# ruc98/Distributed-Data-Parallel-ML-Training

Measured on AMD Instinct MI355X. Metric: images/sec (whole node) VGG-11 CIFAR-10, higher is better.
Workload: dtype bf16; 1 GPU; model=vgg11, global_batch=256, per_gpu_batch=256, parallelism=dp1, hipgraph=True, buckets=1, grad_comm=fp32, comm=inline, optimizer=SGD(lr=0.1, momentum=0.9, wd=1e-4) fused

## Files before the change

distributed-data-parallel-ml-training_amd/csrc/bind.cpp:

```cpp
#include <hip/hip_runtime.h>
#include <pybind11/pybind11.h>
#include <pybind11/stl.h>

#include <stdexcept>
#include <string>
#include <tuple>
#include <vector>

#include "runtime/comm.h"

namespace py = pybind11;
using ddp_amd::BucketSpec;
using ddp_amd::RcclComm;
using ddp_amd::Reducer;

#include "kernels/api.h"

template <typename T>
static T* P(uintptr_t v) { return reinterpret_cast<T*>(v); }
static hipStream_t S(uintptr_t v) { return reinterpret_cast<hipStream_t>(v); }
static void check(int rc, const char* what) {
  if (rc != 0) {
    std::string msg = std::string(what) + " failed: ";
    msg += (rc > 0) ? hipGetErrorString((hipError_t)rc) : "invalid arguments";
// ... 90 lines not shown
      py::tuple b = bn.cast<py::tuple>();
      f.gamma = P<float>(b[0].cast<uintptr_t>());
      f.beta = P<float>(b[1].cast<uintptr_t>());
      f.eps = b[2].cast<float>();
      f.relu = b[3].cast<int>();
      f.pool = b[4].cast<int>();
      f.coef = P<float>(b[5].cast<uintptr_t>());
      f.y = P<unsigned short>(b[6].cast<uintptr_t>());
      f.P = b[7].cast<int>();
      f.Q = b[8].cast<int>();
      fp = &f;
    }
    ddp_amd::TrFwdIn ti{};
    const ddp_amd::TrFwdIn* tp = nullptr;
    if (!fin.is_none()) {
      py::tuple b = fin.cast<py::tuple>();
      ti.z = P<unsigned short>(b[0].cast<uintptr_t>());
      ti.stats = P<float>(b[1].cast<uintptr_t>());
      ti.gamma = P<float>(b[2].cast<uintptr_t>());
      ti.beta = P<float>(b[3].cast<uintptr_t>());
      ti.eps = b[4].cast<float>();
      ti.relu = b[5].cast<int>();
      ti.pool = b[6].cast<int>();
      ti.coef = P<float>(b[7].cast<uintptr_t>());
      ti.y = P<unsigned short>(b[8].cast<uintptr_t>());
      tp = &ti;
    }
    int done = 0;
    const int rc = ddp_conv_fwd_tr(&c, P<void>(x), P<void>(wc), P<float>(bias), P<void>(z),
                                   P<float>(stats), P<float>(ws), ws_elems, fp, &done, tp, S(st));
    if (rc < 0) check(rc, "conv_fwd_tr");
    if (rc >= 2) check(rc - 2, "conv_fwd_tr");
    return rc == 1 ? 1 + done : 0;
  }, py::arg("g"), py::arg("x"), py::arg("wc"), py::arg("bias"), py::arg("z"), py::arg("stats"),
     py::arg("ws"), py::arg("ws_elems"), py::arg("st"), py::arg("bn") = py::none(),
     py::arg("fin") = py::none());
  m.def("l0_ok", [](py::tuple g) {
    auto c = geom(g);
    return ddp_l0_ok(&c) == 1;
  });
  m.def("l0_fwd", [](py::tuple g, uintptr_t x, uintptr_t wc, uintptr_t bias, float eps, int relu,
                     uintptr_t stats, uintptr_t gamma, uintptr_t beta, uintptr_t coef, uintptr_t y,
                     uintptr_t code, uintptr_t zw, uintptr_t st) {
    auto c = geom(g);
    ddp_amd::L0Io io{};
    io.zw = P<void>(zw);
    io.x = P<void>(x); io.wc = P<void>(wc); io.bias = P<float>(bias); io.eps = eps; io.relu = relu;
    io.stats = P<float>(stats); io.gamma = P<float>(gamma); io.beta = P<float>(beta);
    io.coef = P<float>(coef); io.y = P<void>(y); io.code = P<void>(code);
    check(ddp_l0_fwd(&c, &io, S(st)), "l0_fwd");
  });
  m.def("l0_bwd", [](py::tuple g, uintptr_t x, uintptr_t wc, uintptr_t bias, float eps, int relu,
                     uintptr_t coef, uintptr_t dy, uintptr_t sums, uintptr_t dz, uintptr_t dgamma,
                     uintptr_t dbeta, uintptr_t code, uintptr_t zw, uintptr_t st, int sums_ready) {
    auto c = geom(g);
    ddp_amd::L0Io io{};
    io.x = P<void>(x); io.wc = P<void>(wc); io.bias = P<float>(bias); io.eps = eps; io.relu = relu;
    io.coef = P<float>(coef); io.dy = P<void>(dy); io.sums = P<float>(sums); io.dz = P<void>(dz);
    io.dgamma = P<float>(dgamma); io.dbeta = P<float>(dbeta); io.code = P<void>(code);
    io.zw = P<void>(zw);
    io.sums_ready = sums_ready;
    check(ddp_l0_bwd(&c, &io, S(st)), "l0_bwd");
  }, py::arg("g"), py::arg("x"), py::arg("wc"), py::arg("bias"), py::arg("eps"), py::arg("relu"),
     py::arg("coef"), py::arg("dy"), py::arg("sums"), py::arg("dz"), py::arg("dgamma"),
     py::arg("dbeta"), py::arg("code"), py::arg("zw"), py::arg("stream"),
     py::arg("sums_ready") = 0);
  m.def("conv_tr_would_serve", [](py::tuple g, size_t ws_elems, int in_mode) {
    auto c = geom(g);
    return ddp_conv_tr_would_serve(&c, ws_elems, in_mode) == 1;
  });
  m.def("conv_tr_set", [](int mode, int M, int K, int C, int H, int bm, int bn, int splits,
                          int stages) { ddp_conv_tr_set(mode, M, K, C, H, bm, bn, splits, stages); },
        py::arg("mode"), py::arg("M"), py::arg("K"), py::arg("C"), py::arg("H"), py::arg("bm"),
        py::arg("bn"), py::arg("splits"), py::arg("stages") = 0);
  m.def("conv_tr_geometry", [](int BM, int N, int H, int W) {
    int o[7];
    ddp_conv_tr_geometry(BM, N, H, W, o);
    return std::vector<int>(o, o + 7);
  });
  m.def("linear_head_bwd_bn", [](uintptr_t dl, uintptr_t W, uintptr_t x, int B, int F, int J,
                                 uintptr_t g, py::tuple bn, py::tuple bna, uintptr_t dW,
                                 uintptr_t db, uintptr_t st) {
    ddp_amd::BnBwdFuse f{};
    f.z = P<unsigned short>(bn[0].cast<uintptr_t>());
    f.coef = P<float>(bn[1].cast<uintptr_t>());
    f.sums = P<float>(bn[2].cast<uintptr_t>());
    f.pool = bn[3].cast<int>();
    f.relu = bn[4].cast<int>();
    f.Hz = bn[5].cast<int>();
    f.Wz = bn[6].cast<int>();
    ddp_amd::BnBwdApply ap{};
    bn_apply(bna, &ap);
    const int rc = ddp_linear_head_bwd_bn(P<float>(dl), P<float>(W), P<void>(x), B, F, J,
                                          P<float>(g), &f, &ap, P<float>(dW), P<float>(db), S(st));
    if (rc < 0) check(rc, "linear_head_bwd_bn");
    if (rc >= 2) check(rc - 2, "linear_head_bwd_bn");
    return rc == 1;
  });
  m.def("conv_fwd_smallk", [](py::tuple g, uintptr_t x, uintptr_t wc, uintptr_t bias, uintptr_t y,
                              uintptr_t stats, uintptr_t st) {
    auto c = geom(g);
    const int rc = ddp_conv_fwd_smallk(&c, P<void>(x), P<void>(wc), P<float>(bias), P<void>(y),
                                       P<float>(stats), S(st));
    if (rc > 0) check(rc, "conv_fwd_smallk");
    return rc == 0;
  });
  m.def("conv_dgrad", [](py::tuple g, uintptr_t dy, uintptr_t wt, uintptr_t dx, uintptr_t ws,
                         size_t ws_elems, int splits, uintptr_t st, int accumulate, py::object bn,
                         py::object bna, uintptr_t acc_dy, uintptr_t acc_mask) {
    auto c = geom(g);
    if (acc_mask) {
      check(ddp_conv_dgrad_acc(&c, P<void>(dy), P<void>(wt), P<void>(dx), P<float>(ws), ws_elems,
                               splits, P<void>(acc_dy), P<unsigned char>(acc_mask), S(st)),
            "conv_dgrad_acc");
      return false;
    }
    if (bn.is_none()) {
      check(ddp_conv_dgrad(&c, P<void>(dy), P<void>(wt), P<void>(dx), P<float>(ws), ws_elems,
                           splits, accumulate, S(st)), "conv_dgrad");
// ... 490 lines not shown
```

distributed-data-parallel-ml-training_amd/csrc/kernels/api.h:

```cpp
#pragma once
#include <hip/hip_runtime.h>
#include <stddef.h>
#include <stdint.h>

namespace ddp_amd {

#ifdef DDP_AMD_DETERMINISTIC
constexpr int kStatRep = 4096;
constexpr bool kDeterministic = true;
#else
constexpr int kStatRep = 16;
constexpr bool kDeterministic = false;
#endif

struct ConvGeom {
  int N, H, W, C;
  int K;
  int R, S, stride, pad;
  int P, Q;
  int Creal;
  int wkrsc;
};

struct BnArgs {
// ... 61 lines not shown
  const float* beta;
  float eps;
  int relu, pool;
  float* coef;
  unsigned short* y;
};

struct HeadBnIn {
  const unsigned short* z;
  const float* stats;
  const float* gamma;
  const float* beta;
  float eps;
  int relu;
  float* coef;
  unsigned short* y;
};

struct LrSched {
  unsigned step;
  unsigned n;
  unsigned next;
  unsigned pad;
};

struct SgdFuse {
  float* p;
  float* buf;
  unsigned short* wc;
  float lr, momentum, wd, grad_scale;
  int nesterov;
  const LrSched* sched;
};

struct L0Io {
  const void* x;
  const void* wc;
  const float* bias;
  float eps;
  int relu;
  float* stats;
  const float* gamma;
  const float* beta;
  float* coef;
  void* y;
  const void* dy;
  float* sums;
  void* dz;
  void* code;
  void* zw;
  float* dgamma;
  float* dbeta;
  int sums_ready;
};

struct PackDesc {
  const float* p;
  unsigned short* wc;
  unsigned short* wt;
  int K, Cr, C, R, S;
  int krsc;
};

struct AugArgs {
  const unsigned char* images;
  const int* labels;
  const int* indices;
  const int* cursor;
  int L, B, H, W, Cp, pad, flip;
  uint32_t seed, epoch;
  float mean[3], inv_std[3];
  unsigned short* x;
  long long* y;
  float* zero;
  size_t zero_n;
  LrSched* sched;
};

}

extern "C" {
int ddp_conv_fwd(const ddp_amd::ConvGeom* g, const void* x, const void* wc, const float* bias,
                 void* y, float* stats, float* ws, size_t ws_elems, int splits, hipStream_t st);
int ddp_conv_fwd_bn(const ddp_amd::ConvGeom* g, const void* x, const void* wc, const float* bias,
                    void* z, float* stats, float* ws, size_t ws_elems, const ddp_amd::BnFwdFuse* bn,
                    hipStream_t st);
int ddp_conv_fwd_finish(const ddp_amd::ConvGeom* g, float* ws, int splits, const float* bias,
                        void* z, float* stats, const ddp_amd::BnFwdFuse* bn, int* bn_done,
                        hipStream_t st);
int ddp_conv_fwd_tr(const ddp_amd::ConvGeom* g, const void* x, const void* wc, const float* bias,
                    void* z, float* stats, float* ws, size_t ws_elems,
                    const ddp_amd::BnFwdFuse* bn, int* bn_done, const ddp_amd::TrFwdIn* in,
                    hipStream_t st);
int ddp_conv_tr_would_serve(const ddp_amd::ConvGeom* g, size_t ws_elems, int in_mode);
void ddp_conv_tr_set(int mode, int M, int K, int C, int H, int bm, int bn, int splits, int stages);
int ddp_conv_tr_geometry(int BM, int N, int H, int W, int* out7);
int ddp_linear_head_bwd_bn(const float* dl, const float* W, const void* x, int B, int F, int J,
                           const float* gscale, const ddp_amd::BnBwdFuse* bn,
                           const ddp_amd::BnBwdApply* ba, float* dW, float* db, hipStream_t st);
void ddp_conv_bn_fuse_rows(int rows);
int ddp_conv_dgrad(const ddp_amd::ConvGeom* g, const void* dy, const void* wt, void* dx,
                   float* ws, size_t ws_elems, int splits, int accumulate, hipStream_t st);
int ddp_conv_dgrad_acc(const ddp_amd::ConvGeom* g, const void* dy, const void* wt, void* dx,
                       float* ws, size_t ws_elems, int splits, const void* acc_dy,
                       const unsigned char* acc_mask, hipStream_t st);
int ddp_conv_dgrad_bn(const ddp_amd::ConvGeom* g, const void* dy, const void* wt, void* dx,
                      float* ws, size_t ws_elems, int splits, const ddp_amd::BnBwdFuse* bn,
                      const ddp_amd::BnBwdApply* ba, int* bn_done, hipStream_t st);
int ddp_conv_wgrad(const ddp_amd::ConvGeom* g, const void* dy, const void* x, float* dw,
                   float* ws, size_t ws_elems, int splits, hipStream_t st);
int ddp_bn_act_fwd(const ddp_amd::BnArgs* a, hipStream_t st);
int ddp_bn_act_bwd(const ddp_amd::BnArgs* a, hipStream_t st);
int ddp_bn_act_fwd_res(const ddp_amd::BnArgs* a, const ddp_amd::BnArgs* r, hipStream_t st);
int ddp_bn_act_bwd_res(const ddp_amd::BnArgs* a, hipStream_t st);
int ddp_bn_bwd_local_ok(int N, int H, int W, int C, int pool);
void ddp_bn_bwd_local_set(long long max_loads);
int ddp_bn_pool_linear_ce_fwd(const ddp_amd::HeadBnIn* bn, const float* W, const float* b,
                              const long long* labels, int B, int F, int J, float* dlogits,
                              float* loss_sum, int* correct, float* loss_acc, hipStream_t st);
int ddp_linear_ce_fwd(const void* x, const float* W, const float* b, const long long* labels,
                      int B, int F, int J, float* logits, float* dlogits, float* loss_sum,
                      int* correct, float* loss_acc, hipStream_t st);
int ddp_linear_bwd(const float* dlogits, const void* x, const float* W, int B, int F, int J,
                   const float* gscale, void* dx, float* dW, float* db, hipStream_t st);
int ddp_softmax_ce(const void* logits, int logits_bf16, const long long* labels, int B, int J,
                   float* loss_sum, int* correct, void* dlogits, int dlogits_bf16,
                   hipStream_t st);
int ddp_sgd(float* p, const float* g, float* buf, size_t n, float lr, float momentum, float wd,
            float grad_scale, int nesterov, const ddp_amd::LrSched* sched, hipStream_t st);
int ddp_conv_fwd_smallk(const ddp_amd::ConvGeom* g, const void* x, const void* wc,
                        const float* bias, void* y, float* stats, hipStream_t st);
void ddp_conv_options(int stages);
void ddp_conv_epi_stage_set(int on);
int ddp_bn_pool3_fwd(const ddp_amd::BnArgs* a, unsigned char* idx, hipStream_t st);
int ddp_bn_pool3_bwd(const ddp_amd::BnArgs* a, const unsigned char* idx, hipStream_t st);
void ddp_conv_pair_mode(int mode, int items);
void ddp_sgd_fuse_register(float* dw, const ddp_amd::SgdFuse* f, int clear);
void ddp_sgd_fuse_begin();
int ddp_l0_ok(const ddp_amd::ConvGeom* g);
int ddp_l0_fwd(const ddp_amd::ConvGeom* g, const ddp_amd::L0Io* io, hipStream_t st);
int ddp_l0_bwd(const ddp_amd::ConvGeom* g, const ddp_amd::L0Io* io, hipStream_t st);
int ddp_conv_wgrad_final(const ddp_amd::ConvGeom* g, const void* dy, const void* x, float* dw,
                         float* ws, size_t ws_elems, int splits, hipStream_t st);
int ddp_sgd_fuse_taken(uintptr_t* out, int cap);
int ddp_sgd_fuse_taken_master(uintptr_t* out, int cap);
void ddp_conv_pair_force(int splits_dg, int splits_wg, int tile);
int ddp_conv_bwd_pair(const ddp_amd::ConvGeom* g, const void* dy, const void* wc, void* dx,
                      const void* x, float* dw, float* ws, size_t ws_elems,
                      const ddp_amd::BnBwdFuse* bn, const ddp_amd::BnBwdApply* ba, int* bn_done,
                      hipStream_t st);
void ddp_conv_tune_set(int mode, int M, int N, int K, int tile, int splits, int stages);
void ddp_conv_pair_tune_set(int M, int N, int K, int hw, int tile, int sd, int sw);
void ddp_conv_wgrad_pm_set(int on);
void ddp_conv_rows_pm_set(int on);
void ddp_bn_fold_bwd_mb(int mb);
void ddp_bn_fold_grid(int blocks);
int ddp_conv_dense2x2_ok(const ddp_amd::ConvGeom* g);
void ddp_conv_dense2x2_set(int on);
void ddp_conv_tune_clear();
void ddp_conv_force_tile(int tile_plus_one, int stages);
int ddp_pack_conv_weights(const ddp_amd::PackDesc* descs, int n, hipStream_t st);
int ddp_sgd_pack(const void* items, int n_items, const long long* descs, float* p, float* g,
                 float* buf, float lr, float momentum, float wd, float grad_scale, int nesterov,
                 int zero_grad, int* counter, int delta, const unsigned* skip,
                 unsigned short* shadow, float* slot, unsigned* done, unsigned* signal,
                 ddp_amd::LrSched* sched, int sched_advance, hipStream_t st);
int ddp_shard_tail(const void* segs, int n_segs, const float* src, float* dst,
                   const ddp_amd::PackDesc* pack, int n_pack, unsigned* done, unsigned* signal,
                   const unsigned* skip, hipStream_t st);
void ddp_sgd_tile_dims(int RS, int* TK, int* TC);
int ddp_counter_add(int* c, int delta, ddp_amd::LrSched* sched, int sched_mode, hipStream_t st);
int ddp_synth_generate(unsigned char* images, int* labels, int n, int pix_per_img,
                       unsigned int seed, int classes, hipStream_t st);
int ddp_augment(const ddp_amd::AugArgs* a, hipStream_t st);
int ddp_nchw_to_nhwc(const float* x, int N, int C, int H, int W, int Cp, void* out,
                     hipStream_t st);
int ddp_maxpool_fwd(const void* x, int N, int H, int W, int C, int KH, int KW, int stride,
                    int pad, int Ho, int Wo, void* y, void* idx, hipStream_t st);
int ddp_maxpool_bwd(const void* dy, const void* idx, int N, int H, int W, int C, int KH, int KW,
                    int stride, int pad, int Ho, int Wo, void* dx, hipStream_t st);
int ddp_avgpool_fwd(const void* x, int N, int HW, int C, void* y, hipStream_t st);
int ddp_avgpool_bwd(const void* dy, int N, int HW, int C, void* dx, hipStream_t st);
int ddp_colsum(const void* dl, int B, int J, float* db, hipStream_t st);
int ddp_mean_ws(const float* in, size_t n, int ws, float* out, hipStream_t st);
int ddp_scale(float* x, size_t n, float s, hipStream_t st);
int ddp_copy_bytes(void* dst, const void* src, size_t n, hipStream_t st);
int ddp_fill_bytes(void* dst, int value, size_t n, hipStream_t st);
int ddp_comm_standin(float* x, size_t n, int blocks, float usec, float scale, int passes,
                     hipStream_t st);
int ddp_flag_signal(unsigned* flag, hipStream_t st);
int ddp_flag_wait(const unsigned* flag, unsigned* expected, unsigned* err, float timeout_s,
                  hipStream_t st);
int ddp_pack_bf16(const float* x, size_t n, unsigned short* y, hipStream_t st);
int ddp_seg_copy_f32(const void* table, int n, const float* src, float* dst, hipStream_t st);
int ddp_unpack_bf16(const unsigned short* y, size_t n, float* x, hipStream_t st);
}
```

distributed-data-parallel-ml-training_amd/csrc/kernels/conv_igemm.hip:

```cpp
#include "common.h"
#include "api.h"
#include "linear_blocks.h"
#include <algorithm>
#include <map>
#include <set>
#include <cstdlib>

namespace ddp_amd {

enum { MODE_FWD = 0, MODE_DGRAD = 1, MODE_WGRAD = 2 };

typedef short v4i16 __attribute__((ext_vector_type(4)));
typedef short short8_t __attribute__((ext_vector_type(8)));
typedef __attribute__((address_space(3))) v4i16 lds_v4i16;

struct FastDiv {
  unsigned mul;
  int sh;
};
__device__ __forceinline__ int fast_div(int x, FastDiv d) {
  return (int)((__umulhi((unsigned)x, d.mul) + (unsigned)x) >> d.sh);
}
__global__ __launch_bounds__(256) void zero16_kernel(uint4* __restrict__ p, size_t n16) {
  for (size_t i = blockIdx.x * 256ull + threadIdx.x; i < n16; i += (size_t)gridDim.x * 256)
// ... 2558 lines not shown
  }
  const bool l0_sums = d.has_bnf && d.bnf.code != nullptr;
  prep(true);
  const bool fd = needs_finish(MODE_DGRAD, d), fw = needs_finish(MODE_WGRAD, w);
  struct Allow {
    Allow() { g_sgd_allow = true; }
    ~Allow() { g_sgd_allow = false; }
  } allow;
  const ConvArgs dv = finish_view(d, g, MODE_DGRAD);
  if (fd && fw && w.g.wkrsc && bnbwd_fusable(dv)) {
    const WgFinishArgs wa = wg_finish_args(w);
    launch_finish_bnbwd(dv, st, &wa);
  } else if (fd && fw && w.g.wkrsc) {
    int bx, ch;
    dg_finish_grid(dv, &bx, &ch);
    const FinishArgs fa = finish_args(MODE_DGRAD, dv);
    const WgFinishArgs wa = wg_finish_args(w);
    const dim3 grid(bx * ch + wa.gx * wa.gy);
    if (dv.has_bnf)
      hipLaunchKernelGGL(bwd_pair_finish_kernel<true>, grid, dim3(256), 0, st, fa, bx, ch, wa);
    else
      hipLaunchKernelGGL(bwd_pair_finish_kernel<false>, grid, dim3(256), 0, st, fa, bx, ch, wa);
  } else {
    launch_finish<MODE_DGRAD>(dv, st);
    launch_finish<MODE_WGRAD>(w, st);
  }
  if (l0_sums && bn_done) *bn_done = 2;
  return (int)hipGetLastError();
}

extern "C" void ddp_sgd_fuse_register(float* dw, const SgdFuse* f, int clear) {
  if (clear) g_sgd_reg.clear();
  if (dw && f) g_sgd_reg[dw] = *f;
}
extern "C" void ddp_sgd_fuse_begin() {
  g_sgd_taken.clear();
  g_sgd_master.clear();
}
extern "C" int ddp_sgd_fuse_taken_master(uintptr_t* out, int cap) {
  int n = 0;
  for (const float* p : g_sgd_master) {
    if (n < cap) out[n] = reinterpret_cast<uintptr_t>(p);
    ++n;
  }
  return n;
}
extern "C" int ddp_conv_wgrad_final(const ConvGeom* g, const void* dy, const void* x, float* dw,
                                    float* ws, size_t ws_elems, int splits, hipStream_t st) {
  g_sgd_allow = true;
  const int r = ddp_conv_wgrad(g, dy, x, dw, ws, ws_elems, splits, st);
  g_sgd_allow = false;
  return r;
}
extern "C" int ddp_sgd_fuse_taken(uintptr_t* out, int cap) {
  int n = 0;
  for (const float* p : g_sgd_taken) {
    if (n < cap) out[n] = reinterpret_cast<uintptr_t>(p);
    ++n;
  }
  return n;
}
```

distributed-data-parallel-ml-training_amd/csrc/kernels/conv_l0.hip:

```cpp
#include "common.h"
#include "api.h"

#include <algorithm>

namespace ddp_amd {
namespace l0 {

constexpr int kK = 64;
constexpr int kNT = 4;
constexpr int kNKS = 3;

struct Args {
  const unsigned short* x;
  const unsigned short* wc;
  const float* bias;
  int N, H, W, tiles;
  float eps;
  int relu;
  float* stats;
  const float* gamma;
  const float* beta;
  float* coef;
  unsigned short* y;
  const unsigned short* dy;
  float* sums;
  unsigned short* dz;
  unsigned* code;
  unsigned short* zw;
  float* dgamma;
  float* dbeta;
};

typedef unsigned short u16x4 __attribute__((ext_vector_type(4)));

__device__ __forceinline__ bf16x8 as_bf(const uint4& v) { return __builtin_bit_cast(bf16x8, v); }

__device__ __forceinline__ float xor1(float v) { return dpp_f<0xB1>(v); }
__device__ __forceinline__ float xor8(float v) { return dpp_f<0x128>(v); }

struct Tile {
  int n, h, w;
  int hp, wo;
  int d;
};

__device__ __forceinline__ Tile tile_pixel(const Args& a, int t, int rl) {
  const int wb = a.W / 8, per_img = (a.H / 2) * wb;
  Tile p;
  p.n = t / per_img;
  const int rem = t - p.n * per_img;
  p.hp = rem / wb;
  const int cb = rem - p.hp * wb;
  const int r = rl >> 3, c = rl & 7;
  p.h = 2 * p.hp + r;
  p.w = 8 * cb + c;
  p.wo = 4 * cb + (c >> 1);
  p.d = 2 * r + (c & 1);
  return p;
}

constexpr int kRow = 13;
struct Smem {
  uint4 w[kK * kRow];
  float cf[7][kK];
  float red[4][2][kK];
};

__device__ __forceinline__ void stage_weights(const Args& a, Smem& sm) {
  for (int i = threadIdx.x; i < kK * 12; i += 256) {
    const int k = i / 12, tap = i - k * 12;
    sm.w[k * kRow + tap] = tap < 9 ? *reinterpret_cast<const uint4*>(a.wc + ((size_t)k * 9 + tap) * 8)
                                   : make_uint4(0, 0, 0, 0);
  }
}

__device__ __forceinline__ void load_x(const Args& a, const Tile& p, int g, uint4 (&xf)[kNKS]) {
#pragma unroll
  for (int t = 0; t < kNKS; ++t) {
    const int tap = 4 * t + g;
    const int r = tap / 3, s = tap - r * 3;
    const int h = p.h + r - 1, w = p.w + s - 1;
    xf[t] = (tap < 9 && (unsigned)h < (unsigned)a.H && (unsigned)w < (unsigned)a.W)
                ? *reinterpret_cast<const uint4*>(a.x + (((size_t)p.n * a.H + h) * a.W + w) * 8)
// ... 188 lines not shown
          *reinterpret_cast<uint4*>(a.code + win * (kK / 4) + g * 4) =
              make_uint4(cw[0], cw[1], cw[2], cw[3]);
        }
      });
}

__global__ __launch_bounds__(256) void l0_sums_kernel(Args a, int windows) {
  __shared__ float red[256][33];
  const int tid = threadIdx.x, g = tid & 3;
  float mu[kNT][4], is[kNT][4], s1[kNT][4] = {}, s2[kNT][4] = {};
#pragma unroll
  for (int j = 0; j < kNT; ++j)
#pragma unroll
    for (int v = 0; v < 4; ++v) {
      const int c = j * 16 + 4 * g + v;
      mu[j][v] = a.coef[2 * kK + c];
      is[j][v] = a.coef[3 * kK + c];
    }
  for (int w = blockIdx.x * 64 + (tid >> 2); w < windows; w += gridDim.x * 64) {
    const uint4 cq = *reinterpret_cast<const uint4*>(a.code + (size_t)w * (kK / 4) + g * 4);
    const unsigned cw[kNT] = {cq.x, cq.y, cq.z, cq.w};
    u16x4 dv[kNT], zv[kNT];
#pragma unroll
    for (int j = 0; j < kNT; ++j) {
      dv[j] = *reinterpret_cast<const u16x4*>(a.dy + (size_t)w * kK + j * 16 + 4 * g);
      zv[j] = *reinterpret_cast<const u16x4*>(a.zw + (size_t)w * kK + j * 16 + 4 * g);
    }
#pragma unroll
    for (int j = 0; j < kNT; ++j)
#pragma unroll
      for (int v = 0; v < 4; ++v) {
        const float d = ((cw[j] >> (8 * v)) & 0xFFu) < 4u ? bf2f(dv[j][v]) : 0.f;
        s1[j][v] += d;
        s2[j][v] += d * ((bf2f(zv[j][v]) - mu[j][v]) * is[j][v]);
      }
  }
#pragma unroll
  for (int j = 0; j < kNT; ++j)
#pragma unroll
    for (int v = 0; v < 4; ++v) {
      red[tid][j * 4 + v] = s1[j][v];
      red[tid][16 + j * 4 + v] = s2[j][v];
    }
  __syncthreads();
  if (tid < 2 * kK) {
    const int k = tid / kK, c = tid - k * kK;
    const int gg = (c & 15) >> 2, e = k * 16 + (c >> 4) * 4 + (c & 3);
    float t = 0.f;
    for (int i = 0; i < 64; ++i) t += red[4 * i + gg][e];
    atomicAdd(a.sums + stat_rep(blockIdx.x) * 2 * kK + k * kK + c, stat_val(t, blockIdx.x));
  }
}

template <int APPLY>
__global__ __launch_bounds__(256) void l0_bwd_kernel(Args a) {
  __shared__ Smem sm;
  const int lane = threadIdx.x & 63, g = lane >> 4, rl = lane & 15;
  float s1[kNT][4] = {}, s2[kNT][4] = {};
  tile_loop<true>(
      a, g, rl,
      [&] {
        stage_weights(a, sm);
        stage_bias(a, sm);
        if (threadIdx.x < kK) {
          const int c = threadIdx.x;
          const float sc = a.coef[c], mu = a.coef[2 * kK + c], is = a.coef[3 * kK + c];
          sm.cf[0][c] = sc;
          sm.cf[2][c] = is;
          sm.cf[3][c] = -mu * is;
          if (APPLY) {
            const float inv_m = 1.f / ((float)a.N * a.H * a.W);
            float t1 = 0.f, t2 = 0.f;
#pragma unroll
            for (int r = 0; r < kStatRep; ++r) {
              t1 += a.sums[r * 2 * kK + c];
              t2 += a.sums[r * 2 * kK + kK + c];
            }
            const float k1 = t1 * inv_m, k2 = t2 * inv_m;
            sm.cf[4][c] = -sc * k2 * is;
            sm.cf[5][c] = sc * (k2 * is * mu - k1);
            if (blockIdx.x == 0) {
              a.coef[4 * kK + c] = k1;
              a.coef[5 * kK + c] = k2;
              if (a.dgamma) a.dgamma[c] += t2;
              if (a.dbeta) a.dbeta[c] += t1;
            }
          }
        }
      },
      [&](const Tile& cur, const Ops& op) {
        float z[kNT][4];
        conv_z(sm, op.x, g, rl, z);
        const unsigned cw[kNT] = {op.code.x, op.code.y, op.code.z, op.code.w};
        u16x4 o[kNT];
#pragma unroll
        for (int j = 0; j < kNT; ++j)
#pragma unroll
          for (int v = 0; v < 4; ++v) {
            const int c = j * 16 + 4 * g + v;
            const float zf = z[j][v];
            const float dyb = ((cw[j] >> (8 * v)) & 0xFFu) == (unsigned)cur.d ? bf2f(op.dy[j][v]) : 0.f;
            if (APPLY) {
              o[j][v] = f2bf(sm.cf[0][c] * dyb + (zf * sm.cf[4][c] + sm.cf[5][c]));
            } else {
              s1[j][v] += dyb;
              s2[j][v] += dyb * (zf * sm.cf[2][c] + sm.cf[3][c]);
            }
          }
        if (APPLY) {
          unsigned short* dst = a.dz + (((size_t)cur.n * a.H + cur.h) * a.W + cur.w) * kK + 4 * g;
#pragma unroll
          for (int j = 0; j < kNT; ++j) *reinterpret_cast<u16x4*>(dst + j * 16) = o[j];
        }
      });
  if (!APPLY) block_sums(s1, s2, a.sums + stat_rep(blockIdx.x) * 2 * kK, rl, g, sm);
}

static unsigned grid_for(int tiles) {
  return (unsigned)std::max(1, std::min(1024, (tiles + 3) / 4));
}

}
}

using namespace ddp_amd;

static bool l0_shape_ok(const ConvGeom* g) {
  return g->C == 8 && g->Creal <= 8 && g->K == l0::kK && g->R == 3 && g->S == 3 &&
         g->stride == 1 && g->pad == 1 && g->P == g->H && g->Q == g->W && g->H % 2 == 0 &&
         g->W % 8 == 0 && (size_t)g->N * g->H * g->W * l0::kK < (1ull << 31);
}

extern "C" int ddp_l0_ok(const ConvGeom* g) { return l0_shape_ok(g) ? 1 : 0; }

static l0::Args l0_args(const ConvGeom* g, const L0Io* io) {
  l0::Args a{};
  a.x = (const unsigned short*)io->x;
  a.wc = (const unsigned short*)io->wc;
  a.bias = io->bias;
  a.N = g->N; a.H = g->H; a.W = g->W;
  a.tiles = g->N * (g->H / 2) * (g->W / 8);
  a.eps = io->eps;
  a.relu = io->relu;
  a.stats = io->stats;
  a.gamma = io->gamma;
  a.beta = io->beta;
  a.coef = io->coef;
  a.y = (unsigned short*)io->y;
  a.dy = (const unsigned short*)io->dy;
  a.sums = io->sums;
  a.dz = (unsigned short*)io->dz;
  a.code = (unsigned*)io->code;
  a.zw = (unsigned short*)io->zw;
  a.dgamma = io->dgamma;
  a.dbeta = io->dbeta;
  return a;
}

extern "C" int ddp_l0_fwd(const ConvGeom* g, const L0Io* io, hipStream_t st) {
  if (!l0_shape_ok(g) || !io->x || !io->wc || !io->stats || !io->gamma || !io->beta ||
      !io->coef || !io->y || !io->code || !io->zw)
    return -1;
  const l0::Args a = l0_args(g, io);
  const unsigned nb = l0::grid_for(a.tiles);
  hipLaunchKernelGGL(l0::l0_stats_kernel, dim3(nb), dim3(256), 0, st, a);
  hipLaunchKernelGGL(l0::l0_fwd_kernel, dim3(nb), dim3(256), 0, st, a);
  return (int)hipGetLastError();
}

extern "C" int ddp_l0_bwd(const ConvGeom* g, const L0Io* io, hipStream_t st) {
  if (!l0_shape_ok(g) || !io->x || !io->wc || !io->coef || !io->dy || !io->sums || !io->dz ||
      !io->code || !io->zw)
    return -1;
  const l0::Args a = l0_args(g, io);
  const unsigned nb = l0::grid_for(a.tiles);
  const int windows = g->N * (g->H / 2) * (g->W / 2);
  const unsigned ns = (unsigned)std::max(1, std::min(512, (windows + 127) / 128));
  if (!io->sums_ready)
    hipLaunchKernelGGL(l0::l0_sums_kernel, dim3(ns), dim3(256), 0, st, a, windows);
  hipLaunchKernelGGL(l0::l0_bwd_kernel<1>, dim3(nb), dim3(256), 0, st, a);
  return (int)hipGetLastError();
}
```

distributed-data-parallel-ml-training_amd/ops/layers.py:

```python

import torch

from .common import (native, ptr, stream_handle, check, grad_ready, ensure_grad, workspace,
                     step_scratch, weight_krsc, stat_replicas)
from . import common as _common

BF16 = torch.bfloat16
F32 = torch.float32


def _pad8(c):
    return (c + 7) // 8 * 8


class ConvBNActSpec:

    def __init__(self, conv, bn, relu=True, pool=False, cin_pad=None, residual=False):
        K, Cr, R, S = conv.weight.shape
        if conv.groups != 1 or conv.dilation != (1, 1):
            raise ValueError("grouped/dilated conv not supported")
        if conv.stride[0] != conv.stride[1] or conv.padding[0] != conv.padding[1]:
            raise ValueError("only square stride/padding supported")
        if K % 8:
            raise ValueError("output channels must be a multiple of 8")
# ... 173 lines not shown
    native().conv_wgrad(g, ptr(dz), ptr(x), ptr(dweight), ptr(ws), ws.numel(), 0, s,
                        final=int(not need_dx))
    if weight is not None:
        grad_ready([weight])
    if not need_dx:
        return (None, False) if (bna is not None or (bnf is not None and len(bnf) > 7)) else None
    if spec.C != spec.Cr:
        raise RuntimeError("dgrad requested for a channel-padded input layer")
    if (DS_DGRAD_DEFER and link is not None and spec.stride > 1 and link.buf is None
            and link.deferred is None and link.deferred_dgrad is None
            and link.seen + 1 < link.expected):
        link.deferred_dgrad = (g, dz, spec.wc)
        link.seen += 1
        return None
    if link is not None and link.deferred is not None and spec.stride == 1:
        acc_dy, acc_mask = link.deferred
        link.deferred = None
        dx = torch.empty_like(x)
        native().conv_dgrad(g, ptr(dz), ptr(spec.wc), ptr(dx), ptr(ws), ws.numel(), 0, s,
                            accumulate=1, acc_dy=ptr(acc_dy), acc_mask=ptr(acc_mask))
        link.seen += 1
        link.buf = dx
        return link.result()
    if link is not None and link.deferred is not None:
        acc_dy, acc_mask = link.deferred
        link.deferred = None
        link.buf = _masked(acc_dy, acc_mask)
    if link is not None and link.buf is not None:
        native().conv_dgrad(g, ptr(dz), ptr(spec.wc), ptr(link.buf), ptr(ws), ws.numel(), 0, s,
                            accumulate=1)
        link.seen += 1
        return link.result()
    dx = torch.empty_like(x)
    l0_mode = bnf is not None and len(bnf) > 7
    done = native().conv_dgrad(g, ptr(dz), ptr(spec.wc), ptr(dx), ptr(ws), ws.numel(), 0, s,
                               bn=None if l0_mode else bnf, bna=bna)
    if link is not None and link.deferred_dgrad is not None:
        gd, dzd, wcd = link.deferred_dgrad
        link.deferred_dgrad = None
        native().conv_dgrad(gd, ptr(dzd), ptr(wcd), ptr(dx), ptr(ws), ws.numel(), 0, s,
                            accumulate=1)
    if link is not None:
        link.seen += 1
        link.buf = dx
        return link.result()
    if l0_mode:
        return dx, False
    return (dx, bool(done)) if bna is not None else dx


L0_FUSE = True
L0_SUMS_IN_FINISH = True
L0_SUMS_IN_FINISH_MAX_BATCH = 64


def l0_serves(spec, x):
    N, H, W, C = x.shape
    if not (L0_FUSE and x.is_cuda and C == 8 and spec.C == 8 and spec.K == 64 and spec.pool
            and spec.relu and not spec.maxpool3 and not spec.residual):
        return False
    cache = spec.__dict__.setdefault("_l0_cache", {})
    if (N, H, W) not in cache:
        cache[(N, H, W)] = bool(native().l0_ok(spec.geom(N, H, W)))
    return cache[(N, H, W)]


def _defer_bn(spec, residual, running_mean, N, Ho, Wo):
    nxt = spec.next
    if (not FUSE_BN_IN or not CONV_TR or nxt is None or residual is not None
            or running_mean is not None or nxt.C != spec.K or nxt.Cr != nxt.C
            or nxt.R != 3 or nxt.stride != 1 or nxt.pad != 1):
        return False
    if FUSE_BN_IN == 2 and spec.pool and N > FUSE_BN_IN_POOL_MAX_BATCH:
        return False
    if spec.pool and (Ho * 2 != spec._out_p or Wo * 2 != spec._out_q):
        return False
    g = nxt.geom(N, Ho, Wo)
    return bool(native().conv_tr_would_serve(g, workspace(nxt.wc.device).numel(),
                                             2 if spec.pool else 1))


class _ConvPreBNFn(torch.autograd.Function):

    @staticmethod
    def forward(ctx, x, weight, bias, spec, in_link=None):
        spec.maybe_pack()
        spec.dz_fused = None
        spec.deferred = None
        z = conv_forward(spec, x, bias, spec.stats)
        spec.fwd_z = None
        ctx.spec, ctx.in_link = spec, in_link
        ctx.save_for_backward(x, weight, bias)
        return z

    @staticmethod
    def backward(ctx, dz):
        x, weight, bias = ctx.saved_tensors
        if bias is not None:
            ensure_grad(bias)
            grad_ready([bias])
        dx = conv_backward(ctx.spec, x, dz.contiguous(), ensure_grad(weight),
                           ctx.needs_input_grad[0], ctx.in_link, weight=weight)
        return dx, None, None, None, None


def conv_pre_bn(x, spec, in_link=None):
# ... 69 lines not shown
        else:
            z = conv_forward(spec, x, bias, stats, fin=fin)
        spec.fwd_z = z
        ctx.pool3_idx = None
        to_head = (HEAD_BN_FWD and getattr(spec, "defer_to_head", False) and residual is None
                   and rm is None and spec.pool and P == 2 and Q == 2 and spec.relu)
        spec.last_deferred = (not fused and not spec.maxpool3
                              and (to_head or _defer_bn(spec, residual, rm, N, Ho, Wo)))
        if spec.maxpool3:
            idx = torch.empty(N, Ho, Wo, spec.K, dtype=torch.uint8, device=x.device)
            native().bn_pool3_fwd(N, P, Q, spec.K, int(spec.relu), spec.eps, ptr(z), ptr(stats),
                                  ptr(gamma), ptr(beta), ptr(y), ptr(idx), stream_handle(),
                                  ptr(rm), ptr(rv),
                                  float(bn.momentum if bn.momentum is not None else 0.1),
                                  use_running, ptr(spec.coef))
            ctx.pool3_idx = idx
        elif spec.last_deferred:
            spec.deferred = y
        elif not fused:
            mask = None
            if (BN_RELU_MASK and residual is not None and spec.relu and not spec.pool
                    and any(ctx.needs_input_grad) and spec.K % 8 == 0):
                mask = torch.empty(N, P, Q, spec.K // 8, dtype=torch.uint8, device=x.device)
            ctx.relu_mask = mask
            rk = {}
            if res_bn is not None:
                rb = res_bn.bn
                rk = dict(rstats=ptr(res_bn.stats), rgamma=ptr(rb.weight), rbeta=ptr(rb.bias),
                          rcoef=ptr(res_bn.coef), rrunning_mean=ptr(rb.running_mean),
                          rrunning_var=ptr(rb.running_var), reps=res_bn.eps,
                          rmomentum=float(rb.momentum if rb.momentum is not None else 0.1))
            native().bn_act_fwd(N, P, Q, spec.K, int(spec.pool), int(spec.relu), spec.eps, ptr(z),
                                ptr(residual), ptr(stats), ptr(gamma), ptr(beta), ptr(y),
                                stream_handle(), ptr(rm), ptr(rv),
                                float(bn.momentum if bn.momentum is not None else 0.1),
                                use_running, ptr(spec.coef), mask=ptr(mask), **rk)
        ctx.spec = spec
        ctx.has_res = residual is not None
        ctx.in_link, ctx.res_link = in_link, res_link
        ctx.prev_z = spec.prev.fwd_z if spec.prev is not None else None
        ctx.save_for_backward(x, z, stats, weight, bias, gamma, beta, residual)
        return y

    @staticmethod
    def backward(ctx, dy):
        spec = ctx.spec
        x, z, stats, weight, bias, gamma, beta, residual = ctx.saved_tensors
        if ctx.l0:
            N, H, W, _ = x.shape
            dy = dy.contiguous()
            gw, gg, gbt = ensure_grad(weight), ensure_grad(gamma), ensure_grad(beta)
            if bias is not None:
                ensure_grad(bias)
            dz = torch.empty(N, H, W, spec.K, dtype=BF16, device=x.device)
            ready, spec.l0_sums_ready = getattr(spec, "l0_sums_ready", False), False
            native().l0_bwd(spec.geom(N, H, W), ptr(x), ptr(spec.wc), ptr(bias), spec.eps,
                            int(spec.relu), ptr(spec.coef), ptr(dy), ptr(spec.sums), ptr(dz),
                            ptr(gg), ptr(gbt), ptr(ctx.l0_code[0]), ptr(ctx.l0_code[1]),
                            stream_handle(), sums_ready=int(ready))
            ctx.l0_code = None
            spec.l0_code = None
            grad_ready([gamma, beta, bias])
            dx = conv_backward(spec, x, dz, gw, ctx.needs_input_grad[0], ctx.in_link,
                               weight=weight)
            return dx, None, None, None, None, None, None, None, None, None
        N, P, Q, K = z.shape
        sums = spec.sums
        mask = getattr(ctx, "relu_mask", None)
        ctx.relu_mask = None
        defer = (RES_DEFER and mask is not None and ctx.res_link is not None
                 and ctx.needs_input_grad[5] and ctx.res_link.seen == 0
                 and ctx.res_link.buf is None)
        dres = torch.empty_like(z) if (ctx.has_res and ctx.needs_input_grad[5]
                                       and not defer) else None
        gw = ensure_grad(weight)
        gb = ensure_grad(bias) if bias is not None else None
        gg = ensure_grad(gamma)
        gbt = ensure_grad(beta)
        sums_ready, spec.sums_ready = spec.sums_ready, False
        dz_done, spec.dz_fused = spec.dz_fused, None
        spec.fwd_z = None
        if dz_done is not None:
            dz, zref = dz_done
            if zref is None or zref.data_ptr() != z.data_ptr():
                raise RuntimeError("fused BatchNorm backward belongs to another forward pass "
                                   "(stale dz_fused): refusing to use an unwritten gradient")
        elif ctx.pool3_idx is not None:
            dy = dy.contiguous()
            dz = torch.empty_like(z)
            native().bn_pool3_bwd(N, P, Q, K, int(spec.relu), spec.eps, ptr(z), ptr(dy),
                                  ptr(ctx.pool3_idx), ptr(sums), ptr(dz), ptr(gg), ptr(gbt),
                                  stream_handle(), ptr(spec.coef))
            ctx.pool3_idx = None
        elif ctx.res_bn is not None:
            rs, rb = ctx.res_bn, ctx.res_bn.bn
            ctx.res_bn = None
            if mask is None or sums_ready or dz_done is not None:
                raise RuntimeError("shortcut BatchNorm fold needs the forward's ReLU mask")
            dy = dy.contiguous()
            dz = torch.empty_like(z)
            if dres is None:
                dres = torch.empty_like(z)
            rg, rbt = ensure_grad(rb.weight), ensure_grad(rb.bias)
            native().bn_act_bwd(N, P, Q, K, int(spec.pool), int(spec.relu), spec.eps, ptr(z),
                                ptr(residual), ptr(stats), ptr(gamma), ptr(beta), ptr(dy),
                                ptr(sums), ptr(dz), 0, ptr(gg), ptr(gbt), ptr(gb),
                                stream_handle(), ptr(spec.coef), mask=ptr(mask),
                                rcoef=ptr(rs.coef), rsums=ptr(rs.sums), rdz=ptr(dres),
                                rdgamma=ptr(rg), rdbeta=ptr(rbt))
            grad_ready([rb.weight, rb.bias])
        else:
            dy = dy.contiguous()
            dz = torch.empty_like(z)
            native().bn_act_bwd(N, P, Q, K, int(spec.pool), int(spec.relu), spec.eps, ptr(z),
                                0 if mask is not None else ptr(residual), ptr(stats), ptr(gamma),
# ... 292 lines not shown
```

Before: 353,600 images/s.

## Fuse first-layer weight gradient into L0 backward kernel with SGD finish

For the first conv layer, when no input gradient is needed, the backward kernel now computes per-block weight-gradient partials with MFMA directly from the in-register dz and staged input patches, instead of writing dz to memory and running a separate wgrad conv. A finish kernel reduces the per-block slabs and, when available, applies the fused SGD update and repacks bf16 weights. This avoids the dz round-trip and the separate wgrad launch. The cost is extra LDS and register pressure in the backward kernel, which is pinned to four waves per EU.

```diff
diff --git a/distributed-data-parallel-ml-training_amd/csrc/bind.cpp b/distributed-data-parallel-ml-training_amd/csrc/bind.cpp
--- a/distributed-data-parallel-ml-training_amd/csrc/bind.cpp
+++ b/distributed-data-parallel-ml-training_amd/csrc/bind.cpp
@@ -166,7 +166,8 @@
   });
   m.def("l0_bwd", [](py::tuple g, uintptr_t x, uintptr_t wc, uintptr_t bias, float eps, int relu,
                      uintptr_t coef, uintptr_t dy, uintptr_t sums, uintptr_t dz, uintptr_t dgamma,
-                     uintptr_t dbeta, uintptr_t code, uintptr_t zw, uintptr_t st, int sums_ready) {
+                     uintptr_t dbeta, uintptr_t code, uintptr_t zw, uintptr_t st, int sums_ready,
+                     uintptr_t dw, uintptr_t ws, size_t ws_elems) {
     auto c = geom(g);
     ddp_amd::L0Io io{};
     io.x = P<void>(x); io.wc = P<void>(wc); io.bias = P<float>(bias); io.eps = eps; io.relu = relu;
@@ -174,11 +175,15 @@
     io.dgamma = P<float>(dgamma); io.dbeta = P<float>(dbeta); io.code = P<void>(code);
     io.zw = P<void>(zw);
     io.sums_ready = sums_ready;
-    check(ddp_l0_bwd(&c, &io, S(st)), "l0_bwd");
+    io.dw = P<float>(dw); io.ws = P<float>(ws); io.ws_elems = ws_elems;
+    const int rc = ddp_l0_bwd(&c, &io, S(st));
+    if (rc == -2) return 1;
+    check(rc, "l0_bwd");
+    return 0;
   }, py::arg("g"), py::arg("x"), py::arg("wc"), py::arg("bias"), py::arg("eps"), py::arg("relu"),
      py::arg("coef"), py::arg("dy"), py::arg("sums"), py::arg("dz"), py::arg("dgamma"),
      py::arg("dbeta"), py::arg("code"), py::arg("zw"), py::arg("stream"),
-     py::arg("sums_ready") = 0);
+     py::arg("sums_ready") = 0, py::arg("dw") = 0, py::arg("ws") = 0, py::arg("ws_elems") = 0);
   m.def("conv_tr_would_serve", [](py::tuple g, size_t ws_elems, int in_mode) {
     auto c = geom(g);
     return ddp_conv_tr_would_serve(&c, ws_elems, in_mode) == 1;
diff --git a/distributed-data-parallel-ml-training_amd/csrc/kernels/api.h b/distributed-data-parallel-ml-training_amd/csrc/kernels/api.h
--- a/distributed-data-parallel-ml-training_amd/csrc/kernels/api.h
+++ b/distributed-data-parallel-ml-training_amd/csrc/kernels/api.h
@@ -137,6 +137,9 @@
   float* dgamma;
   float* dbeta;
   int sums_ready;
+  float* dw;
+  float* ws;
+  size_t ws_elems;
 };
 
 struct PackDesc {
@@ -228,6 +231,7 @@
 int ddp_conv_wgrad_final(const ddp_amd::ConvGeom* g, const void* dy, const void* x, float* dw,
                          float* ws, size_t ws_elems, int splits, hipStream_t st);
 int ddp_sgd_fuse_taken(uintptr_t* out, int cap);
+int ddp_sgd_fuse_take_final(const float* dw, ddp_amd::SgdFuse* out);
 int ddp_sgd_fuse_taken_master(uintptr_t* out, int cap);
 void ddp_conv_pair_force(int splits_dg, int splits_wg, int tile);
 int ddp_conv_bwd_pair(const ddp_amd::ConvGeom* g, const void* dy, const void* wc, void* dx,
diff --git a/distributed-data-parallel-ml-training_amd/csrc/kernels/conv_igemm.hip b/distributed-data-parallel-ml-training_amd/csrc/kernels/conv_igemm.hip
--- a/distributed-data-parallel-ml-training_amd/csrc/kernels/conv_igemm.hip
+++ b/distributed-data-parallel-ml-training_amd/csrc/kernels/conv_igemm.hip
@@ -2634,6 +2634,12 @@
   g_sgd_allow = false;
   return r;
 }
+extern "C" int ddp_sgd_fuse_take_final(const float* dw, SgdFuse* out) {
+  g_sgd_allow = true;
+  *out = sgd_fuse_for(dw, 1);
+  g_sgd_allow = false;
+  return out->p != nullptr;
+}
 extern "C" int ddp_sgd_fuse_taken(uintptr_t* out, int cap) {
   int n = 0;
   for (const float* p : g_sgd_taken) {
diff --git a/distributed-data-parallel-ml-training_amd/csrc/kernels/conv_l0.hip b/distributed-data-parallel-ml-training_amd/csrc/kernels/conv_l0.hip
--- a/distributed-data-parallel-ml-training_amd/csrc/kernels/conv_l0.hip
+++ b/distributed-data-parallel-ml-training_amd/csrc/kernels/conv_l0.hip
@@ -29,6 +29,7 @@
   unsigned short* zw;
   float* dgamma;
   float* dbeta;
+  float* wg;
 };
 
 typedef unsigned short u16x4 __attribute__((ext_vector_type(4)));
@@ -323,11 +324,40 @@
   }
 }
 
+typedef short v4i16 __attribute__((ext_vector_type(4)));
+typedef __attribute__((address_space(3))) v4i16 lds_v4i16;
+constexpr int kWgN = 28;
+constexpr int kWgSlab = kK * kWgN;
+constexpr int kDzRow = 68;
+struct alignas(16) WgStage {
+  unsigned short dz[16][kDzRow];
+  unsigned short xp[4 * 10][4];
+};
+template <bool ON> struct WgLds { WgStage w[4]; };
+template <> struct WgLds<false> {};
+
 template <int APPLY>
-__global__ __launch_bounds__(256) void l0_bwd_kernel(Args a) {
+__device__ __forceinline__ void l0_bwd_body(const Args& a) {
+  constexpr bool WG = APPLY == 2;
   __shared__ Smem sm;
-  const int lane = threadIdx.x & 63, g = lane >> 4, rl = lane & 15;
+  __shared__ WgLds<WG> wl;
+  const int lane = threadIdx.x & 63, g = lane >> 4, rl = lane & 15, wib = threadIdx.x >> 6;
   float s1[kNT][4] = {}, s2[kNT][4] = {};
+  f32x4 dwacc[kNT][2];
+  int xoff[2] = {0, 0};
+  if (WG) {
+#pragma unroll
+    for (int jt = 0; jt < kNT; ++jt)
+#pragma unroll
+      for (int nt = 0; nt < 2; ++nt) dwacc[jt][nt] = (f32x4){0.f, 0.f, 0.f, 0.f};
+#pragma unroll
+    for (int nt = 0; nt < 2; ++nt) {
+      const int n = nt * 16 + rl;
+      const int tap = n < 27 ? n / 3 : 0, c = n < 27 ? n - tap * 3 : 3;
+      const int tr = tap / 3, ts = tap - tr * 3;
+      xoff[nt] = (((g >> 1) + tr) * 10 + 4 * (g & 1) + ts) * 4 + c;
+    }
+  }
   tile_loop<true>(
       a, g, rl,
       [&] {
@@ -360,6 +390,17 @@
         }
       },
       [&](const Tile& cur, const Ops& op) {
+        if constexpr (WG) {
+          WgStage& st = wl.w[wib];
+#pragma unroll
+          for (int t = 0; t < kNKS; ++t) {
+            const int tap = 4 * t + g;
+            const int tr = tap / 3, ts = tap - tr * 3;
+            if (tap < 9)
+              *reinterpret_cast<uint2*>(st.xp[((rl >> 3) + tr) * 10 + (rl & 7) + ts]) =
+                  make_uint2(op.x[t].x, op.x[t].y);
+          }
+        }
         float z[kNT][4];
         conv_z(sm, op.x, g, rl, z);
         const unsigned cw[kNT] = {op.code.x, op.code.y, op.code.z, op.code.w};
@@ -378,13 +419,119 @@
               s2[j][v] += dyb * (zf * sm.cf[2][c] + sm.cf[3][c]);
             }
           }
-        if (APPLY) {
+        if constexpr (WG) {
+          WgStage& st = wl.w[wib];
+#pragma unroll
+          for (int j = 0; j < kNT; ++j)
+            *reinterpret_cast<u16x4*>(&st.dz[rl][j * 16 + 4 * g]) = o[j];
+          asm volatile("" ::: "memory");
+          const unsigned short* xp = &st.xp[0][0];
+          v4i16 fb[2];
+#pragma unroll
+          for (int nt = 0; nt < 2; ++nt)
+#pragma unroll
+            for (int j = 0; j < 4; ++j) fb[nt][j] = (short)xp[xoff[nt] + 4 * j];
+          const unsigned short* arow = &st.dz[4 * g + (rl >> 2)][4 * (rl & 3)];
+#pragma unroll
+          for (int jt = 0; jt < kNT; ++jt) {
+            const v4i16 fa = __builtin_amdgcn_ds_read_tr16_b64_v4i16((lds_v4i16*)(arow + jt * 16));
+#pragma unroll
+            for (int nt = 0; nt < 2; ++nt)
+              dwacc[jt][nt] =
+                  __builtin_amdgcn_mfma_f32_16x16x16bf16_1k(fa, fb[nt], dwacc[jt][nt], 0, 0, 0);
+          }
+        } else if (APPLY) {
           unsigned short* dst = a.dz + (((size_t)cur.n * a.H + cur.h) * a.W + cur.w) * kK + 4 * g;
 #pragma unroll
           for (int j = 0; j < kNT; ++j) *reinterpret_cast<u16x4*>(dst + j * 16) = o[j];
         }
       });
   if (!APPLY) block_sums(s1, s2, a.sums + stat_rep(blockIdx.x) * 2 * kK, rl, g, sm);
+  if constexpr (WG) {
+    float* red = reinterpret_cast<float*>(sm.w);
+    __syncthreads();
+#pragma unroll
+    for (int w = 0; w < 4; ++w) {
+      if (wib == w) {
+#pragma unroll
+        for (int jt = 0; jt < kNT; ++jt)
+#pragma unroll
+          for (int nt = 0; nt < 2; ++nt)
+#pragma unroll
+            for (int v = 0; v < 4; ++v) {
+              const int e = (jt * 2 + nt) * 4 + v;
+              float t = dwacc[jt][nt][v];
+              if (w > 0) t += red[e * 64 + lane];
+              if (w < 3) {
+                red[e * 64 + lane] = t;
+              } else if (nt * 16 + rl < kWgN) {
+                a.wg[(size_t)blockIdx.x * kWgSlab + (jt * 16 + 4 * g + v) * kWgN + nt * 16 + rl] = t;
+              }
+            }
+      }
+      if (w < 3) __syncthreads();
+    }
+  }
+}
+
+template <int APPLY>
+__global__ __launch_bounds__(256) void l0_bwd_kernel(Args a) {
+  l0_bwd_body<APPLY>(a);
+}
+template <>
+__global__ __launch_bounds__(256) __attribute__((amdgpu_waves_per_eu(4, 4))) void l0_bwd_kernel<2>(
+    Args a) {
+  l0_bwd_body<2>(a);
+}
+
+constexpr int kWgBatch = 8;
+__global__ __launch_bounds__(256) void l0_wgrad_finish_kernel(const float* __restrict__ ws,
+                                                              int nslab, float* __restrict__ dw,
+                                                              int wkrsc, SgdFuse sg) {
+  __shared__ float4 red[64][4];
+  const bool opt = sg.p != nullptr;
+  const float lr = opt ? sched_lr_block(sg.sched, sg.lr) : sg.lr;
+  const int e = threadIdx.x & 3, s0 = threadIdx.x >> 2;
+  const int i4 = blockIdx.x * 4 + e;
+  float4 v = make_float4(0.f, 0.f, 0.f, 0.f);
+  for (int z = s0; z < nslab; z += 64 * kWgBatch) {
+    float4 t[kWgBatch];
+#pragma unroll
+    for (int u = 0; u < kWgBatch; ++u)
+      if (z + 64 * u < nslab)
+        t[u] = reinterpret_cast<const float4*>(ws + (size_t)(z + 64 * u) * kWgSlab)[i4];
+#pragma unroll
+    for (int u = 0; u < kWgBatch; ++u)
+      if (z + 64 * u < nslab) { v.x += t[u].x; v.y += t[u].y; v.z += t[u].z; v.w += t[u].w; }
+  }
+  red[s0][e] = v;
+  for (int h = 32; h >= 1; h >>= 1) {
+    __syncthreads();
+    if (s0 < h) {
+      const float4 o = red[s0 + h][e];
+      v.x += o.x; v.y += o.y; v.z += o.z; v.w += o.w;
+      red[s0][e] = v;
+    }
+  }
+  if (s0 != 0) return;
+  const float vv[4] = {v.x, v.y, v.z, v.w};
+#pragma unroll
+  for (int t = 0; t < 4; ++t) {
+    const int idx = i4 * 4 + t, k = idx / kWgN, n = idx - k * kWgN;
+    if (n >= 27) continue;
+    const int tap = n / 3, c = n - tap * 3;
+    if (opt) {
+      const int mi = k * 27 + n;
+      float b = sg.buf[mi];
+      const float np = sgd_update1(sg.p[mi], vv[t], b, lr, sg.momentum, sg.wd, sg.grad_scale,
+                                   sg.nesterov);
+      sg.p[mi] = np;
+      sg.buf[mi] = b;
+      sg.wc[(k * 9 + tap) * 8 + c] = f2bf(np);
+    } else {
+      dw[wkrsc ? k * 27 + n : (k * 3 + c) * 9 + tap] += vv[t];
+    }
+  }
 }
 
 static unsigned grid_for(int tiles) {
@@ -440,15 +587,26 @@
 }
 
 extern "C" int ddp_l0_bwd(const ConvGeom* g, const L0Io* io, hipStream_t st) {
-  if (!l0_shape_ok(g) || !io->x || !io->wc || !io->coef || !io->dy || !io->sums || !io->dz ||
-      !io->code || !io->zw)
+  const bool fused = !io->dz && io->dw;
+  if (!l0_shape_ok(g) || !io->x || !io->wc || !io->coef || !io->dy || !io->sums ||
+      (!io->dz && !io->dw) || !io->code || !io->zw)
     return -1;
-  const l0::Args a = l0_args(g, io);
+  l0::Args a = l0_args(g, io);
   const unsigned nb = l0::grid_for(a.tiles);
+  if (fused && (g->Creal != 3 || !io->ws || io->ws_elems < (size_t)nb * l0::kWgSlab)) return -2;
   const int windows = g->N * (g->H / 2) * (g->W / 2);
   const unsigned ns = (unsigned)std::max(1, std::min(512, (windows + 127) / 128));
   if (!io->sums_ready)
     hipLaunchKernelGGL(l0::l0_sums_kernel, dim3(ns), dim3(256), 0, st, a, windows);
-  hipLaunchKernelGGL(l0::l0_bwd_kernel<1>, dim3(nb), dim3(256), 0, st, a);
+  if (!fused) {
+    hipLaunchKernelGGL(l0::l0_bwd_kernel<1>, dim3(nb), dim3(256), 0, st, a);
+    return (int)hipGetLastError();
+  }
+  a.wg = io->ws;
+  hipLaunchKernelGGL(l0::l0_bwd_kernel<2>, dim3(nb), dim3(256), 0, st, a);
+  SgdFuse sg{};
+  if (g->wkrsc) ddp_sgd_fuse_take_final(io->dw, &sg);
+  hipLaunchKernelGGL(l0::l0_wgrad_finish_kernel, dim3(l0::kWgSlab / 16), dim3(256), 0, st,
+                     (const float*)io->ws, (int)nb, io->dw, g->wkrsc, sg);
   return (int)hipGetLastError();
 }
diff --git a/distributed-data-parallel-ml-training_amd/ops/layers.py b/distributed-data-parallel-ml-training_amd/ops/layers.py
--- a/distributed-data-parallel-ml-training_amd/ops/layers.py
+++ b/distributed-data-parallel-ml-training_amd/ops/layers.py
@@ -249,6 +249,7 @@
 L0_FUSE = True
 L0_SUMS_IN_FINISH = True
 L0_SUMS_IN_FINISH_MAX_BATCH = 64
+L0_WGRAD_FUSE = True
 
 
 def l0_serves(spec, x):
@@ -424,15 +425,25 @@
             gw, gg, gbt = ensure_grad(weight), ensure_grad(gamma), ensure_grad(beta)
             if bias is not None:
                 ensure_grad(bias)
-            dz = torch.empty(N, H, W, spec.K, dtype=BF16, device=x.device)
             ready, spec.l0_sums_ready = getattr(spec, "l0_sums_ready", False), False
-            native().l0_bwd(spec.geom(N, H, W), ptr(x), ptr(spec.wc), ptr(bias), spec.eps,
-                            int(spec.relu), ptr(spec.coef), ptr(dy), ptr(spec.sums), ptr(dz),
-                            ptr(gg), ptr(gbt), ptr(ctx.l0_code[0]), ptr(ctx.l0_code[1]),
-                            stream_handle(), sums_ready=int(ready))
+            args = (ptr(x), ptr(spec.wc), ptr(bias), spec.eps, int(spec.relu), ptr(spec.coef),
+                    ptr(dy), ptr(spec.sums))
+            tail = (ptr(gg), ptr(gbt), ptr(ctx.l0_code[0]), ptr(ctx.l0_code[1]), stream_handle())
+            fused = L0_WGRAD_FUSE and not ctx.needs_input_grad[0]
+            if fused:
+                ws = workspace(x.device)
+                fused = not native().l0_bwd(spec.geom(N, H, W, weight_krsc(gw)), *args, 0, *tail,
+                                            sums_ready=int(ready), dw=ptr(gw), ws=ptr(ws),
+                                            ws_elems=ws.numel())
+            if not fused:
+                dz = torch.empty(N, H, W, spec.K, dtype=BF16, device=x.device)
+                native().l0_bwd(spec.geom(N, H, W), *args, ptr(dz), *tail, sums_ready=int(ready))
             ctx.l0_code = None
             spec.l0_code = None
             grad_ready([gamma, beta, bias])
+            if fused:
+                grad_ready([weight])
+                return (None,) * 10
             dx = conv_backward(spec, x, dz, gw, ctx.needs_input_grad[0], ctx.in_link,
                                weight=weight)
             return dx, None, None, None, None, None, None, None, None, None
```

After: 367,800 images/s (median of 6 runs). 4.0% higher.
